# LorienLV/genarchbench

Measured on AMD Instinct MI355X. Metric: bsw ROI M alignments/sec, higher is better.
Workload: dtype i16/i32; 1 GPU; bsw-large; total_items=10000000

## Files before the change

### genarchbench_amd/csrc/bsw.hip

```cpp
#include "gab_internal.h"
#include <atomic>
#include <algorithm>
#include <new>
#include <string.h>
#include <time.h>
#include <stdlib.h>

namespace {

constexpr int kQBuckets = 256;
constexpr int kTBuckets = 256;
constexpr int kNumKeys = kQBuckets * kTBuckets;
constexpr int kClassStep = 16;
constexpr int kNumClasses = kQBuckets / kClassStep;

struct BswConst {
    int32_t o_del, e_del, o_ins, e_ins, zdrop, end_bonus, w, max_sc;
    uint32_t row_lo[5];
    uint32_t row_hi[5];
};

struct BswStats {
    unsigned long long cells;
    int32_t max_h0[kNumClasses];
    int32_t bad;
    int32_t first_bad;
};
GAB_STATIC_ATOMIC64(BswStats, cells);

struct BswIO {
    const uint8_t *ref; const int64_t *ref_off;
    const uint8_t *qry; const int64_t *qry_off;
    const int32_t *len1, *len2, *h0;
    int64_t ref_bytes, qry_bytes, n;
    int64_t ref_lo, qry_lo;
    int64_t ref_hi, qry_hi;
};

__device__ __forceinline__ int bsw_key(int qlen, int tlen, int h0) {
    int tb = tlen >> 3; if (tb > kTBuckets / 4 - 1) tb = kTBuckets / 4 - 1;
    int hc = h0 >> 5; if (hc > 3) hc = 3;
    return (qlen - 1) * kTBuckets + tb * 4 + hc;
}

__device__ __forceinline__ int bsw_hslot(int key) { return (int)(((uint32_t)key * 4099u) & (uint32_t)(kNumKeys - 1)); }
static_assert((kNumKeys & (kNumKeys - 1)) == 0, "bsw_hslot needs a power-of-two key space");

__global__ __launch_bounds__(256) void bsw_hist(BswIO io, uint32_t *hist, uint32_t *rank, BswStats *st) {
    __shared__ int cls_h0[kNumClasses];
    if (threadIdx.x < kNumClasses) cls_h0[threadIdx.x] = 0;
    __syncthreads();
    int64_t i = (int64_t)blockIdx.x * blockDim.x + threadIdx.x;
    int64_t stride = (int64_t)gridDim.x * blockDim.x;
    for (; i < io.n; i += stride) {
        int ql = io.len2[i], tl = io.len1[i], h = io.h0[i];
        int64_t ro = io.ref_off[i], qo = io.qry_off[i];
        bool ok = ql >= 1 && ql <= GAB_BSW_MAX_QLEN && tl >= 1 && tl <= GAB_BSW_MAX_TLEN && h >= 0 &&
                  h <= (1 << 29) && ro >= io.ref_lo && qo >= io.qry_lo &&
                  ro + tl + 3 <= io.ref_bytes && qo + ql + 3 <= io.qry_bytes &&
                  ro + tl <= io.ref_hi && qo + ql <= io.qry_hi;
        if (!ok) {
            atomicAdd(&st->bad, 1);
            atomicMin((unsigned int *)&st->first_bad, (unsigned int)(i + 1 > 0x7fffffff ? 0x7fffffff : i + 1));
            rank[i] = ~0u;
            continue;
        }
        if (h > 0) atomicMax(&cls_h0[(ql - 1) / kClassStep], h);
        rank[i] = atomicAdd(&hist[bsw_hslot(bsw_key(ql, tl, h))], 1u);
    }
    __syncthreads();
    if (threadIdx.x < kNumClasses && cls_h0[threadIdx.x] > 0) atomicMax(&st->max_h0[threadIdx.x], cls_h0[threadIdx.x]);
}

constexpr int kScanBlocks = kNumKeys / 1024;
static_assert(kScanBlocks == 64, "bsw_scan_b reduces the block totals with one wave");
__global__ __launch_bounds__(1024) void bsw_scan_a(const uint32_t *__restrict__ hist, uint32_t *__restrict__ start, uint32_t *__restrict__ sums) {
    __shared__ uint32_t wsum[16];
    const int t = threadIdx.x, key = blockIdx.x * 1024 + t, lane = t & 63, wv = t >> 6;
    const uint32_t v = hist[bsw_hslot(key)];
    uint32_t inc = v;
    for (int o = 1; o < 64; o <<= 1) { const uint32_t u = __shfl_up(inc, o); if (lane >= o) inc += u; }
    if (lane == 63) wsum[wv] = inc;
    __syncthreads();
    uint32_t before = 0;
    for (int k = 0; k < wv; k++) before += wsum[k];
    start[key] = before + inc - v;
    if (t == 1023) sums[blockIdx.x] = before + inc;
}
__global__ __launch_bounds__(1024) void bsw_scan_b(uint32_t *__restrict__ start, const uint32_t *__restrict__ sums, uint32_t *__restrict__ qstart) {
    __shared__ uint32_t s_off, s_total;
    const int t = threadIdx.x, key = blockIdx.x * 1024 + t;
    if (t < 64) {
        const uint32_t sv = sums[t];
        uint32_t mine = t < (int)blockIdx.x ? sv : 0, all = sv;
        for (int o = 32; o > 0; o >>= 1) { mine += __shfl_xor(mine, o); all += __shfl_xor(all, o); }
        if (t == 0) { s_off = mine; s_total = all; }
    }
    __syncthreads();
    const uint32_t run = start[key] + s_off;
    start[key] = run;
    if ((key % kTBuckets) == 0) qstart[key / kTBuckets] = run;
    if (key == kNumKeys - 1) { start[kNumKeys] = s_total; qstart[kQBuckets] = s_total; }
}

struct __attribute__((aligned(32))) BswRec { int64_t ref_off, qry_off; int32_t len1, len2, h0; uint32_t id; };

__global__ __launch_bounds__(256) void bsw_scatter(BswIO io, const uint32_t *__restrict__ start, const uint32_t *__restrict__ rank,
                                                   BswRec *recs) {
    int64_t i = (int64_t)blockIdx.x * blockDim.x + threadIdx.x;
    int64_t stride = (int64_t)gridDim.x * blockDim.x;
    for (; i < io.n; i += stride) {
        int ql = io.len2[i], tl = io.len1[i];
        if (rank[i] == ~0u) continue;
        BswRec r;
        r.ref_off = io.ref_off[i]; r.qry_off = io.qry_off[i]; r.len1 = tl; r.len2 = ql; r.h0 = io.h0[i]; r.id = (uint32_t)i;
        recs[start[bsw_key(ql, tl, r.h0)] + rank[i]] = r;
    }
}

__device__ __forceinline__ uint32_t load_u32_unaligned(const uint8_t *p) {
    uint32_t w;
    __builtin_memcpy(&w, p, 4);
    return w;
}

template <bool WIDE>
__global__ __launch_bounds__(64) void bsw_dp(BswIO io, BswConst c, const BswRec *__restrict__ recs,
                                            int64_t kbeg, int64_t kend, int qcap,
                                            int32_t *__restrict__ score_out,
                                            gab_bsw_result *__restrict__ result_out, BswStats *st) {
    extern __shared__ uint32_t lds[];
    const int lane = threadIdx.x;
    const int64_t k = kbeg + (int64_t)(gridDim.x - 1 - blockIdx.x) * 64 + lane;
    const bool valid = k < kend;
    BswRec rec; rec.ref_off = rec.qry_off = 0; rec.len1 = rec.len2 = rec.h0 = 0; rec.id = 0u;
    if (valid) rec = recs[k];
    const uint32_t id = rec.id;

    uint32_t *const H = lds + lane;
    uint32_t *const E = lds + (size_t)(qcap + 1) * 64 + lane;
    uint8_t *const QC = reinterpret_cast<uint8_t *>(lds + (size_t)(WIDE ? 2 : 1) * (qcap + 1) * 64) + lane * 4;

    unsigned long long cells = 0;
    if (valid) {
        const int qlen = rec.len2, tlen = rec.len1, h0 = rec.h0;
        const uint8_t *q = io.qry + rec.qry_off;
        const uint8_t *t = io.ref + rec.ref_off;
        const int oe_del = c.o_del + c.e_del, oe_ins = c.o_ins + c.e_ins;
        const int e_del = c.e_del, e_ins = c.e_ins;

        for (int w4 = 0; w4 * 4 < qlen; w4++)
            *reinterpret_cast<uint32_t *>(QC + w4 * 256) = load_u32_unaligned(q + w4 * 4);

        int w = c.w;
        {
            int lim = (int)((double)(qlen * c.max_sc + c.end_bonus - c.o_ins) / e_ins + 1.);
            lim = lim > 1 ? lim : 1; w = w < lim ? w : lim;
            lim = (int)((double)(qlen * c.max_sc + c.end_bonus - c.o_del) / e_del + 1.);
            lim = lim > 1 ? lim : 1; w = w < lim ? w : lim;
        }
        const bool score_only = result_out == nullptr;
        bool prune = score_only && (qlen <= w + 1 || h0 - oe_ins - (w + 1) * e_ins <= 0) && (c.zdrop == 0 || c.zdrop >= 8 * c.max_sc);
        int best, best_i, best_j, g_i, gscore, max_off;
      for (;;) {
// ... 512 lines not shown
                    uint32_t cl2 = (uint32_t)(qlen - 2 * pb) | (uint32_t)(qlen - 2 * pb - 1) << 16;
                    uint32_t acc = 0;
                    for (int p = pb; p <= pe; p++, cl2 -= 0x00020002u) {
                        uint32_t d2 = CW[p * 64] & 0x00ff00ffu;
                        if (p == pb && (beg & 1)) d2 &= 0xffff0000u;
                        if (p == pe && !(end & 1)) d2 &= 0x0000ffffu;
                        const uint32_t gain = pk_mul_lo(pk_min_u16(cl2, r2), m2);
                        acc = pk_max_i16(acc, pk_mul_lo(add_u32_v(d2, gain), pk_min_u16_1(d2)));
                    }
                    bound = max(bound, max((int)(acc & 0xffffu), (int)(acc >> 16)));
                }
                stop = bound <= best;
            }
            if (stop) break;
        }
        if (!SO || !abandon) break;
        prune = false;
      }
        score_out[id] = best;
        if constexpr (!SO) {
            gab_bsw_result r;
            r.score = best; r.qle = best_j + 1; r.tle = best_i + 1;
            r.gtle = g_i + 1; r.gscore = gscore; r.max_off = max_off;
            result_out[id] = r;
        }
    }
#undef CELL16
#undef QPAIR
    for (int o = 32; o > 0; o >>= 1) cells += __shfl_xor(cells, o);
    if (lane == 0 && cells) atomicAdd(&st->cells, cells);
}

using BswDp8Fn = void (*)(BswIO, BswConst, const BswRec *, int64_t, int64_t, int, int32_t *, gab_bsw_result *, BswStats *);
template <bool SYM, bool MS1> BswDp8Fn bsw_dp8_pick(bool so) { return so ? bsw_dp8<SYM, MS1, true> : bsw_dp8<SYM, MS1, false>; }
BswDp8Fn bsw_dp8_kernel(bool sym, bool ms1, bool so) {
    return sym ? (ms1 ? bsw_dp8_pick<true, true>(so) : bsw_dp8_pick<true, false>(so))
               : (ms1 ? bsw_dp8_pick<false, true>(so) : bsw_dp8_pick<false, false>(so));
}

}

struct gab_bsw {
    gab_tuning tun = gab_tuning_loaded();
    gab_host_stream hs;
    int device = 0;
    gab_bsw_params prm;
    BswConst cst;
    gab_devbuf ws;
    gab_devbuf io;
    hipEvent_t ev[4] = {nullptr, nullptr, nullptr, nullptr};
    static constexpr int kAux = 1;
    hipStream_t aux[kAux] = {nullptr};
    hipEvent_t fork = nullptr, join[kAux] = {nullptr};
    bool have_stats = false;
    uint32_t *h_qstart = nullptr;
    BswStats *h_stats = nullptr;
    int64_t last_cells = 0;
    bool out_of_order = false;
};

extern "C" int gab_bsw_create(const gab_bsw_params *p, int device, gab_bsw **out) {
    if (!p || !out) { gab_set_error("gab_bsw_create: NULL argument"); return GAB_EINVAL; }
    *out = nullptr;
    GAB_CHECK(p->e_del > 0 && p->e_ins > 0 && p->o_del >= 0 && p->o_ins >= 0,
              "gab_bsw_create: gap penalties must be o>=0, e>0 (got o_del=%d e_del=%d o_ins=%d e_ins=%d)",
              p->o_del, p->e_del, p->o_ins, p->e_ins);
    GAB_CHECK(p->w >= 0 && p->zdrop >= 0, "gab_bsw_create: w and zdrop must be >= 0");
    GAB_CHECK(p->o_del + p->e_del < 32768 && p->o_ins + p->e_ins < 32768 && p->end_bonus >= -32768 &&
              p->end_bonus < 32768, "gab_bsw_create: penalties out of 16-bit range");
    int rc = gab_check_device(device);
    if (rc) return rc;
    gab_device_guard g(device);
    gab_bsw *h = new (std::nothrow) gab_bsw();
    if (!h) { gab_set_error("out of host memory"); return GAB_ENOMEM; }
    h->device = device; h->prm = *p;
    BswConst &c = h->cst;
    c.o_del = p->o_del; c.e_del = p->e_del; c.o_ins = p->o_ins; c.e_ins = p->e_ins;
    c.zdrop = p->zdrop; c.end_bonus = p->end_bonus; c.w = p->w;
    int mx = 0;
    for (int k = 0; k < 25; k++) mx = p->mat[k] > mx ? p->mat[k] : mx;
    c.max_sc = mx;
    for (int t = 0; t < 5; t++) {
        uint32_t lo = 0;
        for (int q = 0; q < 4; q++) lo |= (uint32_t)(uint8_t)(p->mat[t * 5 + q] + 128) << (8 * q);
        c.row_lo[t] = lo;
        c.row_hi[t] = (uint32_t)(uint8_t)(p->mat[t * 5 + 4] + 128);
    }
    for (int k = 0; k < 4; k++)
        if (hipEventCreate(&h->ev[k]) != hipSuccess) { gab_set_error("hipEventCreate failed"); delete h; return GAB_EDEVICE; }
    bool aux_ok = hipEventCreateWithFlags(&h->fork, hipEventDisableTiming) == hipSuccess;
    for (int k = 0; k < gab_bsw::kAux && aux_ok; k++)
        aux_ok = hipStreamCreateWithFlags(&h->aux[k], hipStreamNonBlocking) == hipSuccess &&
                 hipEventCreateWithFlags(&h->join[k], hipEventDisableTiming) == hipSuccess;
    if (!aux_ok) { gab_set_error("gab_bsw_create: stream / event creation failed"); delete h; return GAB_EDEVICE; }
    if (hipFuncSetAttribute((const void *)bsw_dp<false>, hipFuncAttributeMaxDynamicSharedMemorySize, 160 * 1024) != hipSuccess ||
        hipFuncSetAttribute((const void *)bsw_dp<true>, hipFuncAttributeMaxDynamicSharedMemorySize, 160 * 1024) != hipSuccess) {
        gab_set_error("hipFuncSetAttribute(MaxDynamicSharedMemorySize) failed"); delete h; return GAB_EDEVICE;
    }
    for (int k = 0; k < 8; k++)
        if (hipFuncSetAttribute((const void *)bsw_dp8_kernel(k & 4, k & 2, k & 1), hipFuncAttributeMaxDynamicSharedMemorySize, 160 * 1024 - 64) != hipSuccess) {
            gab_set_error("hipFuncSetAttribute(MaxDynamicSharedMemorySize) failed"); delete h; return GAB_EDEVICE;
        }
    if (hipHostMalloc((void **)&h->h_qstart, sizeof(uint32_t) * (kQBuckets + 1)) != hipSuccess ||
        hipHostMalloc((void **)&h->h_stats, sizeof(BswStats)) != hipSuccess) {
        gab_set_error("hipHostMalloc failed"); delete h; return GAB_ENOMEM;
    }
    *out = h;
    return GAB_OK;
}

extern "C" void gab_bsw_destroy(gab_bsw *h) {
    if (!h) return;
    gab_device_guard g(h->device);
    h->ws.release(); h->io.release(); h->hs.release();
    for (int k = 0; k < 4; k++) if (h->ev[k]) (void)hipEventDestroy(h->ev[k]);
    if (h->fork) (void)hipEventDestroy(h->fork);
    for (int k = 0; k < gab_bsw::kAux; k++) {
        if (h->join[k]) (void)hipEventDestroy(h->join[k]);
        if (h->aux[k]) (void)hipStreamDestroy(h->aux[k]);
    }
    if (h->h_qstart) (void)hipHostFree(h->h_qstart);
    if (h->h_stats) (void)hipHostFree(h->h_stats);
    delete h;
}

static int bsw_run_device_impl(gab_bsw *h, const uint8_t *ref, int64_t ref_bytes, const int64_t *ref_off,
                               const uint8_t *qry, int64_t qry_bytes, const int64_t *qry_off,
                               const int32_t *len1, const int32_t *len2, const int32_t *h0, int64_t n,
                               int32_t *score_out, gab_bsw_result *result_out, void *stream_, int64_t ref_lo, int64_t qry_lo,
                               int64_t ref_hi, int64_t qry_hi);
extern "C" int gab_bsw_run_device(gab_bsw *h, const uint8_t *ref, int64_t ref_bytes, const int64_t *ref_off,
                                  const uint8_t *qry, int64_t qry_bytes, const int64_t *qry_off,
                                  const int32_t *len1, const int32_t *len2, const int32_t *h0, int64_t n,
                                  int32_t *score_out, gab_bsw_result *result_out, void *stream_) {
    if (h) gab_tuning_refresh(&h->tun);
    return bsw_run_device_impl(h, ref, ref_bytes, ref_off, qry, qry_bytes, qry_off, len1, len2, h0, n, score_out, result_out, stream_, 0, 0,
                               ref_bytes, qry_bytes);
}
static int bsw_run_device_impl(gab_bsw *h, const uint8_t *ref, int64_t ref_bytes, const int64_t *ref_off,
                               const uint8_t *qry, int64_t qry_bytes, const int64_t *qry_off,
                               const int32_t *len1, const int32_t *len2, const int32_t *h0, int64_t n,
                               int32_t *score_out, gab_bsw_result *result_out, void *stream_, int64_t ref_lo, int64_t qry_lo,
                               int64_t ref_hi, int64_t qry_hi) {
    GAB_CHECK(h, "gab_bsw_run_device: NULL handle");
    GAB_CHECK(n >= 0 && n < (1ll << 31), "gab_bsw_run_device: n=%lld out of range", (long long)n);
    h->have_stats = false;
    if (n == 0) return GAB_OK;
    GAB_CHECK(ref && ref_off && qry && qry_off && len1 && len2 && h0 && score_out,
              "gab_bsw_run_device: NULL buffer");
    gab_device_guard g(h->device);
    hipStream_t s = (hipStream_t)stream_;

    const size_t o_hist = 0;
    const size_t o_start = o_hist + sizeof(uint32_t) * kNumKeys;
    const size_t o_qstart = o_start + sizeof(uint32_t) * (kNumKeys + 1);
    const size_t o_sums = o_qstart + sizeof(uint32_t) * (kQBuckets + 1);
    const size_t o_stats = (o_sums + sizeof(uint32_t) * kScanBlocks + 15) & ~(size_t)15;
    const size_t o_recs = (o_stats + sizeof(BswStats) + 255) & ~(size_t)255;
    const size_t o_rank = o_recs + ((sizeof(BswRec) * (size_t)n + 255) & ~(size_t)255);
    int rc = h->ws.reserve(o_rank + sizeof(uint32_t) * (size_t)n);
    if (rc) return rc;
    char *base = h->ws.as<char>();
    uint32_t *d_hist = (uint32_t *)(base + o_hist), *d_start = (uint32_t *)(base + o_start);
    uint32_t *d_qstart = (uint32_t *)(base + o_qstart);
    BswStats *d_stats = (BswStats *)(base + o_stats);
    BswRec *d_recs = (BswRec *)(base + o_recs);
    uint32_t *d_rank = (uint32_t *)(base + o_rank);

    BswIO io{ref, ref_off, qry, qry_off, len1, len2, h0, ref_bytes, qry_bytes, n, ref_lo, qry_lo, ref_hi, qry_hi};
    GAB_HIP(hipEventRecord(h->ev[0], s));
    GAB_HIP(hipMemsetAsync(base, 0, o_recs, s));
    {
        BswStats init; memset(&init, 0, sizeof(init)); init.first_bad = 0x7fffffff;
        *h->h_stats = init;
        GAB_HIP(hipMemcpyAsync(d_stats, h->h_stats, sizeof(BswStats), hipMemcpyHostToDevice, s));
    }
    int grid = (int)(gab_ceil_div(n, 256) < 1024 ? gab_ceil_div(n, 256) : 1024);
    hipLaunchKernelGGL(bsw_hist, dim3(grid), dim3(256), 0, s, io, d_hist, d_rank, d_stats);
    hipLaunchKernelGGL(bsw_scan_a, dim3(kScanBlocks), dim3(1024), 0, s, d_hist, d_start, (uint32_t *)(base + o_sums));
    hipLaunchKernelGGL(bsw_scan_b, dim3(kScanBlocks), dim3(1024), 0, s, d_start, (const uint32_t *)(base + o_sums), d_qstart);
    hipLaunchKernelGGL(bsw_scatter, dim3(grid), dim3(256), 0, s, io, d_start, d_rank, d_recs);
    GAB_HIP(hipMemcpyAsync(h->h_qstart, d_qstart, sizeof(uint32_t) * (kQBuckets + 1), hipMemcpyDeviceToHost, s));
    GAB_HIP(hipMemcpyAsync(h->h_stats, d_stats, sizeof(BswStats), hipMemcpyDeviceToHost, s));
    GAB_HIP(hipStreamSynchronize(s));
    if (h->h_stats->bad) {
        gab_set_error("gab_bsw_run_device: %d pair(s) violate the limits (first: pair %d): need 1<=len2<=%d, "
                      "1<=len1<=%d, 0<=h0, offsets inside the slabs with 3 more readable bytes behind every sequence",
                      h->h_stats->bad, h->h_stats->first_bad - 1, GAB_BSW_MAX_QLEN, GAB_BSW_MAX_TLEN);
        return GAB_EINVAL;
    }
    int max_h0 = 0;
    for (int cls = 0; cls < kNumClasses; cls++) max_h0 = h->h_stats->max_h0[cls] > max_h0 ? h->h_stats->max_h0[cls] : max_h0;
    const bool sym = h->cst.o_del + h->cst.e_del == h->cst.o_ins + h->cst.e_ins;
    const bool ms1 = h->cst.max_sc <= 1;

    GAB_HIP(hipEventRecord(h->ev[1], s));
    GAB_HIP(hipEventRecord(h->fork, s));
    for (int k = 0; k < gab_bsw::kAux; k++) GAB_HIP(hipStreamWaitEvent(h->aux[k], h->fork, 0));
    int nlaunch = 0;
    hipStream_t s_main = s;
    const bool one_launch = n <= (int64_t)64 * 8192;
    int top_cls = kNumClasses - 1;
    while (top_cls > 0 && h->h_qstart[(top_cls + 1) * kClassStep] <= h->h_qstart[top_cls * kClassStep]) top_cls--;
    for (int cls = kNumClasses - 1; cls >= 0; cls--) {
        int64_t kb = h->h_qstart[cls * kClassStep], ke = h->h_qstart[(cls + 1) * kClassStep];
        if (one_launch) { if (cls != top_cls) continue; kb = 0; }
        if (ke <= kb) continue;
        const int qcap = (cls + 1) * kClassStep;
        const int blocks = (int)gab_ceil_div(ke - kb, 64);
        s = (nlaunch % (gab_bsw::kAux + 1)) ? h->aux[nlaunch % (gab_bsw::kAux + 1) - 1] : s_main;
        nlaunch++;
        const int64_t hmax = (int64_t)(one_launch ? max_h0 : h->h_stats->max_h0[cls]) + (int64_t)qcap * h->cst.max_sc;
        const bool wide = hmax > 32767;
        if (h->tun.bsw_trace)
            fprintf(stderr, "[gab_bsw_dp %p] class %d qcap %d pairs %lld bits %d sym %d ms1 %d\n", (void *)h, cls, qcap,
                    (long long)(ke - kb), hmax <= 255 ? 8 : wide ? 32 : 16, (int)sym, (int)ms1);
        if (hmax <= 255 && h->cst.max_sc >= 0) {
            const size_t lds8 = sizeof(uint32_t) * 64 * ((size_t)(qcap + 2) / 2 + ((size_t)(qcap + 1) / 2 + 3) / 4 + 1);
            auto kern = bsw_dp8_kernel(sym, ms1, result_out == nullptr);
            hipLaunchKernelGGL(kern, dim3(blocks), dim3(64), lds8, s, io, h->cst, d_recs, kb, ke, qcap,
                               score_out, result_out, d_stats);
            continue;
        }
        const size_t lds = sizeof(uint32_t) * 64 * ((size_t)(wide ? 2 : 1) * (qcap + 1) + (size_t)(qcap + 3) / 4);
        if (wide)
            hipLaunchKernelGGL(bsw_dp<true>, dim3(blocks), dim3(64), lds, s, io, h->cst, d_recs, kb, ke, qcap,
                               score_out, result_out, d_stats);
        else
            hipLaunchKernelGGL(bsw_dp<false>, dim3(blocks), dim3(64), lds, s, io, h->cst, d_recs, kb, ke, qcap,
                               score_out, result_out, d_stats);
    }
    s = s_main;
    GAB_HIP(hipGetLastError());
    for (int k = 0; k < gab_bsw::kAux; k++) {
        GAB_HIP(hipEventRecord(h->join[k], h->aux[k]));
        GAB_HIP(hipStreamWaitEvent(s, h->join[k], 0));
    }
    GAB_HIP(hipEventRecord(h->ev[2], s));
    GAB_HIP(hipMemcpyAsync(h->h_stats, d_stats, sizeof(BswStats), hipMemcpyDeviceToHost, s));
    GAB_HIP(hipEventRecord(h->ev[3], s));
    h->have_stats = true;
    return GAB_OK;
}

extern "C" int gab_bsw_run(gab_bsw *h, const uint8_t *ref, const int64_t *ref_off, const uint8_t *qry,
                           const int64_t *qry_off, const int32_t *len1, const int32_t *len2,
                           const int32_t *h0, int64_t n, int32_t *score_out) {
    GAB_CHECK(h, "gab_bsw_run: NULL handle");
    GAB_CHECK(n >= 0 && n < (1ll << 31), "gab_bsw_run: n=%lld out of range", (long long)n);
    if (n == 0) return GAB_OK;
    GAB_CHECK(ref && ref_off && qry && qry_off && len1 && len2 && h0 && score_out, "gab_bsw_run: NULL buffer");
    gab_device_guard g(h->device);
    gab_tuning_refresh(&h->tun);
    const bool trace = h->tun.bsw_trace;
    const double t_0 = gab_now_ms();
    int64_t rb = 0, qb = 0, ra = INT64_MAX, qa = INT64_MAX;
    auto take = [&](int64_t i) {
        int64_t r = ref_off[i] + len1[i], q = qry_off[i] + len2[i];
        rb = r > rb ? r : rb; qb = q > qb ? q : qb;
        ra = ref_off[i] < ra ? ref_off[i] : ra; qa = qry_off[i] < qa ? qry_off[i] : qa;
        return ref_off[i] >= 0 && qry_off[i] >= 0 && len1[i] >= 0 && len2[i] >= 0;
    };
    bool sampled = n > 4096 && !h->out_of_order && !h->tun.bsw_full_scan;
    if (sampled) {
        bool ok = take(0);
        ok = take(n - 1) && ok;
        for (int k = 1; k <= 64; k++) ok = take((n - 1) * k / 65) && ok;
        if (!ok || rb - ra > 65536 * n || qb - qa > 65536 * n) sampled = false;
    }
    if (!sampled) {
        rb = qb = 0; ra = qa = INT64_MAX;
        for (int64_t i = 0; i < n; i++)
            GAB_CHECK(take(i), "gab_bsw_run: negative offset/length at pair %lld", (long long)i);
    }
    ra &= ~(int64_t)255; qa &= ~(int64_t)255;
    const size_t rpad = ((size_t)(rb - ra) + 3 + 255) & ~(size_t)255, qpad = ((size_t)(qb - qa) + 3 + 255) & ~(size_t)255;
    const size_t nn = (size_t)n;
    size_t o = 0;
    const size_t o_ref = o; o += rpad;
    const size_t o_qry = o; o += qpad;
    const size_t o_roff = o; o += 8 * nn;
    const size_t o_qoff = o; o += 8 * nn;
    const size_t o_l1 = o; o += 4 * nn;
    const size_t o_l2 = o; o += 4 * nn;
    const size_t o_h0 = o; o += 4 * nn;
    const size_t o_sc = o; o += 4 * nn;
    int rc = h->io.reserve(o);
    if (rc) return rc;
    char *b = h->io.as<char>();
    hipStream_t s = nullptr;
    if ((rc = h->hs.get(&s)) != GAB_OK) return rc;
    const double t_1 = gab_now_ms();
    {
        std::lock_guard<std::mutex> gate(gab_h2d_mutex(h->device));
        GAB_HIP(hipMemcpyAsync(b + o_ref, ref + ra, (size_t)(rb - ra), hipMemcpyHostToDevice, s));
        GAB_HIP(hipMemcpyAsync(b + o_qry, qry + qa, (size_t)(qb - qa), hipMemcpyHostToDevice, s));
        GAB_HIP(hipMemcpyAsync(b + o_roff, ref_off, 8 * nn, hipMemcpyHostToDevice, s));
        GAB_HIP(hipMemcpyAsync(b + o_qoff, qry_off, 8 * nn, hipMemcpyHostToDevice, s));
        GAB_HIP(hipMemcpyAsync(b + o_l1, len1, 4 * nn, hipMemcpyHostToDevice, s));
        GAB_HIP(hipMemcpyAsync(b + o_l2, len2, 4 * nn, hipMemcpyHostToDevice, s));
        GAB_HIP(hipMemcpyAsync(b + o_h0, h0, 4 * nn, hipMemcpyHostToDevice, s));
        GAB_HIP(hipStreamSynchronize(s));
    }
    double t_2 = 0;
    if (trace) { GAB_HIP(hipStreamSynchronize(s)); t_2 = gab_now_ms(); }
    rc = bsw_run_device_impl(h, (const uint8_t *)(b + o_ref) - ra, ra + (int64_t)rpad, (const int64_t *)(b + o_roff),
                             (const uint8_t *)(b + o_qry) - qa, qa + (int64_t)qpad, (const int64_t *)(b + o_qoff),
                             (const int32_t *)(b + o_l1), (const int32_t *)(b + o_l2), (const int32_t *)(b + o_h0),
                             n, (int32_t *)(b + o_sc), nullptr, s, ra, qa, rb, qb);
    if (rc == GAB_EINVAL && sampled) {
        h->out_of_order = true;
        return gab_bsw_run(h, ref, ref_off, qry, qry_off, len1, len2, h0, n, score_out);
    }
    if (rc) return rc;
    double t_3 = 0;
    if (trace) { GAB_HIP(hipStreamSynchronize(s)); t_3 = gab_now_ms(); }
    GAB_HIP(hipMemcpyAsync(score_out, b + o_sc, 4 * nn, hipMemcpyDeviceToHost, s));
    GAB_HIP(hipStreamSynchronize(s));
    if (trace)
        fprintf(stderr, "[gab_bsw_run %p] %lld pairs: host scan %.2f ms, H2D of %.1f MB %.2f ms, sort + DP %.2f ms, D2H %.2f ms\n", (void *)h,
                (long long)n, t_1 - t_0, (double)((rb - ra) + (qb - qa) + 28 * n) / 1e6, t_2 - t_1, t_3 - t_2, gab_now_ms() - t_3);
    return GAB_OK;
}

extern "C" int gab_bsw_reserve(gab_bsw *h, int64_t max_pairs, int64_t max_ref_bytes, int64_t max_qry_bytes) {
    GAB_CHECK(h, "gab_bsw_reserve: NULL handle");
    GAB_CHECK(max_pairs >= 0 && max_pairs < (1ll << 31) && max_ref_bytes >= 0 && max_qry_bytes >= 0, "gab_bsw_reserve: size out of range");
    gab_device_guard g(h->device);
    const size_t nn = (size_t)max_pairs;
    int rc = h->io.reserve(std::max<size_t>((((size_t)max_ref_bytes + 3 + 511) & ~(size_t)255) + (((size_t)max_qry_bytes + 3 + 511) & ~(size_t)255) + 32 * nn + 1024,
                                            (size_t)4 << 20));
    if (rc) return rc;
    rc = h->ws.reserve(sizeof(uint32_t) * (2 * kNumKeys + kQBuckets + 4) + sizeof(BswStats) + 1024 + (sizeof(BswRec) + sizeof(uint32_t)) * nn);
    if (rc) return rc;
    hipStream_t s = nullptr;
    if ((rc = h->hs.get(&s)) != GAB_OK) return rc;
    GAB_HIP(hipMemsetAsync(h->io.p, 0, h->io.cap, s));
    GAB_HIP(hipMemsetAsync(h->ws.p, 0, h->ws.cap, s));
    GAB_HIP(hipStreamSynchronize(s));
    if ((rc = gab_warm_copy_engines(s, h->io.p, h->io.cap)) != GAB_OK) return rc;
    static const uint8_t seq[40] = {0, 1, 2, 3, 0, 1, 2, 3, 3, 2, 1, 0, 0, 1, 2, 3, 0, 1, 2, 3, 3, 2, 1, 0, 0, 1, 2, 3, 0, 1, 2, 3, 3, 2, 1, 0, 0, 0, 0, 0};
    const int64_t ro[2] = {0, 4}, qo[2] = {2, 8};
    const int32_t l1[2] = {24, 20}, l2[2] = {20, 16}, h0[2] = {10, 0};
    int32_t sc[2];
    const bool had = h->have_stats;
    rc = gab_bsw_run(h, seq, ro, seq, qo, l1, l2, h0, 2, sc);
    h->have_stats = had;
    return rc;
}

extern "C" int gab_bsw_last_stats(gab_bsw *h, int64_t *cells, float *kernel_ms, float *total_ms) {
    GAB_CHECK(h, "gab_bsw_last_stats: NULL handle");
    GAB_CHECK(h->have_stats, "gab_bsw_last_stats: no completed run on this handle");
    gab_device_guard g(h->device);
    GAB_HIP(hipEventSynchronize(h->ev[3]));
    if (cells) *cells = (int64_t)h->h_stats->cells;
    if (kernel_ms) GAB_HIP(hipEventElapsedTime(kernel_ms, h->ev[1], h->ev[2]));
    if (total_ms) GAB_HIP(hipEventElapsedTime(total_ms, h->ev[0], h->ev[3]));
    return GAB_OK;
}
```

### genarchbench_amd/csrc/gab_core.hip

```cpp
#define GAB_NO_COPY_MACROS
#include "gab_internal.h"
#include <string.h>
#include <stdlib.h>
#include <algorithm>
#include <mutex>
#include <unordered_set>

static thread_local char g_err[512] = "";

void gab_set_error(const char *fmt, ...) {
    va_list ap;
    va_start(ap, fmt);
    vsnprintf(g_err, sizeof(g_err), fmt, ap);
    va_end(ap);
}

extern "C" const char *gab_version(void) { return "gab-hip 0.1 (gfx950)"; }

#include <execinfo.h>
#include <fcntl.h>
#include <signal.h>
#include <sys/stat.h>
#include <unistd.h>
namespace {
// ... 29 lines not shown
}
extern "C" const char *gab_last_error(void) { return g_err; }

extern "C" int gab_device_count(void) {
    int n = 0;
    if (hipGetDeviceCount(&n) != hipSuccess) return 0;
    return n;
}

extern "C" int gab_device_pci_bus_id(int device, char *buf, int len) {
    if (!buf || len < 16) { gab_set_error("gab_device_pci_bus_id: buffer of at least 16 bytes needed"); return GAB_EINVAL; }
    buf[0] = 0;
    const int n = gab_device_count();
    if (n <= 0) { gab_set_error("no HIP device visible"); return GAB_ENODEV; }
    if (device < 0 || device >= n) { gab_set_error("device %d out of range (0..%d)", device, n - 1); return GAB_EINVAL; }
    GAB_HIP(hipDeviceGetPCIBusId(buf, len, device));
    return GAB_OK;
}

int gab_check_device(int device) {
    int n = gab_device_count();
    if (n <= 0) {
        gab_set_error("no HIP device visible (libgab_hip has no CPU fallback)");
        return GAB_ENODEV;
    }
    if (device < 0 || device >= n) {
        gab_set_error("device %d out of range (0..%d)", device, n - 1);
        return GAB_EINVAL;
    }
    hipDeviceProp_t prop;
    if (hipGetDeviceProperties(&prop, device) != hipSuccess) {
        gab_set_error("hipGetDeviceProperties(%d) failed", device);
        return GAB_EDEVICE;
    }
    if (const char *e = getenv("GAB_HIP_SCHEDULE")) {
        static std::once_flag once;
        std::call_once(once, [e] {
            (void)hipSetDeviceFlags(!strcmp(e, "spin") ? hipDeviceScheduleSpin : !strcmp(e, "yield") ? hipDeviceScheduleYield : hipDeviceScheduleBlockingSync);
        });
    }
    if (strncmp(prop.gcnArchName, "gfx950", 6) != 0) {
        gab_set_error("device %d is %s; this library is built for gfx950 only", device, prop.gcnArchName);
        return GAB_ENODEV;
    }
    return GAB_OK;
}

bool gab_tuning_live() { const char *e = getenv("GAB_TUNING_LIVE"); return e && *e && atoi(e) != 0; }
void gab_tuning_load(gab_tuning *t) {
    *t = gab_tuning();
    auto on = [](const char *name) { return getenv(name) != nullptr; };
    auto num = [](const char *name, long long unset) { const char *e = getenv(name); return e ? atoll(e) : unset; };
    t->bsw_trace = on("GAB_BSW_TRACE"); t->bsw_full_scan = on("GAB_BSW_FULL_SCAN");
    t->bpm_score64 = on("GAB_BPM_SCORE64"); t->bitpal_no_bv = on("GAB_BITPAL_NO_BV"); t->bpm_slices = (int)num("GAB_BPM_SLICES", 0);
    t->bpm_trace = on("GAB_BPM_TRACE");
    if (const char *e = getenv("GAB_WFA_TUNE")) {
        t->wfa_tuned = true;
        const int k = sscanf(e, "%d,%d,%d,%d,%d,%d,%d", &t->wfa_tune[0], &t->wfa_tune[1], &t->wfa_tune[2], &t->wfa_tune[3], &t->wfa_tune[4], &t->wfa_tune[5], &t->wfa_tune[6]);
        t->wfa_tune_fields = k > 0 ? k : 0;
    }
    t->wfa_no_static = on("GAB_WFA_NO_STATIC"); t->wfa_trace = on("GAB_WFA_TRACE");
    t->wfa_pool2 = (int)num("GAB_WFA_POOL2", -1); t->wfa_slots = (int)num("GAB_WFA_SLOTS", -1);
    if (const char *e = getenv("GAB_CHAIN_HELPERS")) { t->chain_helpers_set = true; t->chain_helpers = atoi(e); }
    { const char *e = getenv("GAB_CHAIN_KERNEL"); t->chain_walk = e && !strcmp(e, "walk"); }
    t->chain_trace = on("GAB_CHAIN_TRACE"); t->chain_feed_giveup = on("GAB_CHAIN_FEED_GIVEUP"); t->chain_fed_serial = on("GAB_CHAIN_FED_SERIAL");
    t->chain_no_overlap = on("GAB_CHAIN_NO_OVERLAP"); t->chain_no_feed = on("GAB_CHAIN_NO_FEED");
    if (const char *e = getenv("GAB_CHAIN_TAB")) t->chain_tab = atoi(e) != 0;
    t->chain_tab_min = num("GAB_CHAIN_TAB_MIN", -1); t->chain_fast_min = num("GAB_CHAIN_FAST_MIN", -1); t->chain_fast_calls = num("GAB_CHAIN_FAST_CALLS", -1);
    t->chain_feed_min = num("GAB_CHAIN_FEED_MIN", -1); t->chain_tab_mb = num("GAB_CHAIN_TAB_MB", -1);
    if (const char *e = getenv("GAB_CHAIN_GATHER_MASK")) { strncpy(t->chain_gather_mask, e, sizeof t->chain_gather_mask - 1); t->chain_gather_mask[sizeof t->chain_gather_mask - 1] = 0; }
    t->chain_gather_blocks = (int)num("GAB_CHAIN_GATHER_BLOCKS", 0);
    t->fmi_lds_entries = (int)num("GAB_FMI_LDS_ENTRIES", 0); t->fmi_waves = (int)num("GAB_FMI_WAVES", 0); t->fmi_wide = (int)num("GAB_FMI_WIDE", 1);
    t->fmi_wide_cap = (int)num("GAB_FMI_WIDE_CAP", 0); t->fmi_kmer_depth = (int)num("GAB_FMI_KMER_DEPTH", -1);
    t->fmi_wide_lists = num("GAB_FMI_WIDE_LISTS", 0) != 0; t->fmi_debug = on("GAB_FMI_DEBUG");
    t->fmi_batch = num("GAB_FMI_BATCH", 0); t->fmi_scratch_mb = num("GAB_FMI_SCRATCH_MB", 0);
    t->kmer_part_floor = num("GAB_KMER_PART_FLOOR", 0) != 0;
    t->abea_trace_bytes = num("GAB_ABEA_TRACE_BYTES", 0);
}

extern "C" int gab_device_alloc(int device, size_t bytes, void **out) {
    if (!out) { gab_set_error("gab_device_alloc: NULL argument"); return GAB_EINVAL; }
    *out = nullptr;
    int rc = gab_check_device(device);
    if (rc) return rc;
    gab_device_guard g(device);
    GAB_HIP(hipMalloc(out, bytes ? bytes : 1));
    return GAB_OK;
}
extern "C" void gab_device_free(int device, void *p) {
    if (!p) return;
    gab_device_guard g(device);
    (void)hipFree(p);
}
extern "C" int gab_device_copy_to_host(int device, void *dst, const void *d_src, size_t bytes) {
    if (bytes == 0) return GAB_OK;
    if (!dst || !d_src) { gab_set_error("gab_device_copy_to_host: NULL argument"); return GAB_EINVAL; }
    gab_device_guard g(device);
    GAB_HIP(gab_memcpy_async(dst, d_src, bytes, hipMemcpyDeviceToHost, nullptr));
    GAB_HIP(hipStreamSynchronize(nullptr));
    return GAB_OK;
}

static std::mutex g_host_mu;
static std::unordered_set<void *> &gab_host_blocks() { static std::unordered_set<void *> s; return s; }
extern "C" int gab_host_alloc(size_t bytes, void **out) {
    if (!out) { gab_set_error("gab_host_alloc: NULL argument"); return GAB_EINVAL; }
// ... 123 lines not shown
```

### genarchbench_amd/csrc/gab_internal.h

```cpp
#pragma once
#include <hip/hip_runtime.h>
#include <stdint.h>
#include <stdarg.h>
#include <stdio.h>
#include <stddef.h>
#include <time.h>
#include <mutex>
#include "../../include/gab.h"

void gab_set_error(const char *fmt, ...);

#define GAB_HIP(call)                                                                    \
    do {                                                                                 \
        hipError_t e_ = (call);                                                          \
        if (e_ != hipSuccess) {                                                          \
            gab_set_error("%s:%d: %s -> %s", __FILE__, __LINE__, #call,                  \
                          hipGetErrorString(e_));                                        \
            return e_ == hipErrorOutOfMemory ? GAB_ENOMEM : GAB_EDEVICE;                 \
        }                                                                                \
    } while (0)

#define GAB_CHECK(cond, ...)                                                             \
    do {                                                                                 \
        if (!(cond)) {                                                                   \
// ... 4 lines not shown

struct gab_devbuf {
    void *p = nullptr;
    size_t cap = 0;
    int reserve(size_t bytes) {
        if (bytes <= cap) return GAB_OK;
        if (p) (void)hipFree(p);
        p = nullptr; cap = 0;
        size_t want = bytes + bytes / 8 + 256;
        hipError_t e = hipMalloc(&p, want);
        if (e != hipSuccess) {
            gab_set_error("hipMalloc(%zu) failed: %s", want, hipGetErrorString(e));
            p = nullptr;
            return GAB_ENOMEM;
        }
        cap = want;
        return GAB_OK;
    }
    void release() { if (p) (void)hipFree(p); p = nullptr; cap = 0; }
    template <typename T> T *as() const { return reinterpret_cast<T *>(p); }
};

struct gab_device_guard {
    int prev = -1; bool changed = false;
    explicit gab_device_guard(int dev) {
        if (hipGetDevice(&prev) == hipSuccess && prev != dev) { changed = (hipSetDevice(dev) == hipSuccess); }
    }
    ~gab_device_guard() { if (changed) (void)hipSetDevice(prev); }
};

struct gab_host_stream {
    hipStream_t s = nullptr;
    int get(hipStream_t *out) {
        if (!s && hipStreamCreateWithFlags(&s, hipStreamNonBlocking) != hipSuccess) {
            s = nullptr; gab_set_error("hipStreamCreateWithFlags failed: %s", hipGetErrorString(hipGetLastError()));
            return GAB_EDEVICE;
        }
        *out = s;
        return GAB_OK;
    }
    void release() { if (s) (void)hipStreamDestroy(s); s = nullptr; }
};

std::mutex &gab_h2d_mutex(int device);
int gab_warm_copy_engines(hipStream_t s, void *dev, size_t dev_bytes);
int gab_check_device(int device);
bool gab_is_pinned(const void *p);

static inline int64_t gab_ceil_div(int64_t a, int64_t b) { return (a + b - 1) / b; }
static inline double gab_now_ms() { timespec ts; clock_gettime(CLOCK_MONOTONIC, &ts); return ts.tv_sec * 1e3 + ts.tv_nsec * 1e-6; }

struct gab_tuning {
    bool bsw_trace = false, bsw_full_scan = false;
    bool bpm_score64 = false, bitpal_no_bv = false, bpm_trace = false;
    int bpm_slices = 0;
    bool wfa_tuned = false, wfa_no_static = false, wfa_trace = false;
    int wfa_tune[7] = {0, 0, 0, 0, 0, 0, 0};
    int wfa_tune_fields = 0;
    int wfa_pool2 = -1, wfa_slots = -1;
    int chain_helpers = 0;
    bool chain_helpers_set = false, chain_walk = false, chain_trace = false, chain_feed_giveup = false, chain_fed_serial = false;
    bool chain_no_overlap = false, chain_no_feed = false;
    int chain_tab = -1;
    long long chain_tab_min = -1, chain_fast_min = -1, chain_fast_calls = -1, chain_feed_min = -1, chain_tab_mb = -1;
    char chain_gather_mask[32] = "";
    int chain_gather_blocks = 0;
    int fmi_lds_entries = 0, fmi_waves = 0, fmi_wide = 1, fmi_wide_cap = 0, fmi_kmer_depth = -1;
    bool fmi_wide_lists = false, fmi_debug = false;
    long long fmi_batch = 0, fmi_scratch_mb = 0;
    bool kmer_part_floor = false;
    long long abea_trace_bytes = 0;
};
void gab_tuning_load(gab_tuning *t);
bool gab_tuning_live();
inline void gab_tuning_refresh(gab_tuning *t) { if (gab_tuning_live()) gab_tuning_load(t); }
inline gab_tuning gab_tuning_loaded() { gab_tuning t; gab_tuning_load(&t); return t; }

#define GAB_CHECK_ATOMIC64(off) GAB_CHECK((((size_t)(off)) & 7) == 0, "internal error: a 64-bit atomic at offset %zu of a scratch layout (not a multiple of 8)", (size_t)(off))
#define GAB_STATIC_ATOMIC64(type, member) static_assert(offsetof(type, member) % 8 == 0 && alignof(type) >= 8, "64-bit atomics need 8-byte alignment: " #type "::" #member)

__device__ __forceinline__ uint32_t gab_wave_slot(uint32_t *counter, bool active) {
    const unsigned long long m = __ballot(active);
    if (!m) return 0;
    const int lane = (int)(threadIdx.x & 63u);
    const int leader = __builtin_ctzll(m);
    uint32_t base = 0;
    if (lane == leader) base = atomicAdd(counter, (uint32_t)__popcll(m));
    base = __shfl(base, leader);
    return base + (uint32_t)__popcll(m & ((1ull << lane) - 1ull));
}

hipError_t gab_memcpy_async(void *dst, const void *src, size_t bytes, hipMemcpyKind kind, hipStream_t s);
hipError_t gab_memcpy(void *dst, const void *src, size_t bytes, hipMemcpyKind kind);
#ifndef GAB_NO_COPY_MACROS
#define hipMemcpyAsync gab_memcpy_async
#define hipMemcpy gab_memcpy
#endif
```

Baseline: 400.1 M alignments/s.

## Slice BSW input and overlap second slice's sort with first slice's DP

```diff
diff --git a/genarchbench_amd/csrc/bsw.hip b/genarchbench_amd/csrc/bsw.hip
--- a/genarchbench_amd/csrc/bsw.hip
+++ b/genarchbench_amd/csrc/bsw.hip
@@ -13,6 +13,11 @@
 constexpr int kNumKeys = kQBuckets * kTBuckets;
 constexpr int kClassStep = 16;
 constexpr int kNumClasses = kQBuckets / kClassStep;
+constexpr int kSlices = 2;
+constexpr int64_t kSlice0 = 1 << 20;
+constexpr int64_t kSliceMin = 1 << 22;
+constexpr int kSortGridBeside = 256;
+static_assert(kSliceMin >= (1 << 21) && kSlice0 < kSliceMin && kSlice0 >= 64 * 8192, "slice 0 has to fill the chip with its class launches, and calls below 2^21 pairs stay unsliced");
 
 struct BswConst {
     int32_t o_del, e_del, o_ins, e_ins, zdrop, end_bonus, w, max_sc;
@@ -46,13 +51,13 @@
 __device__ __forceinline__ int bsw_hslot(int key) { return (int)(((uint32_t)key * 4099u) & (uint32_t)(kNumKeys - 1)); }
 static_assert((kNumKeys & (kNumKeys - 1)) == 0, "bsw_hslot needs a power-of-two key space");
 
-__global__ __launch_bounds__(256) void bsw_hist(BswIO io, uint32_t *hist, uint32_t *rank, BswStats *st) {
+__global__ __launch_bounds__(256) void bsw_hist(BswIO io, int64_t lo, int64_t hi, uint32_t *hist, uint32_t *rank, BswStats *st) {
     __shared__ int cls_h0[kNumClasses];
     if (threadIdx.x < kNumClasses) cls_h0[threadIdx.x] = 0;
     __syncthreads();
-    int64_t i = (int64_t)blockIdx.x * blockDim.x + threadIdx.x;
+    int64_t i = lo + (int64_t)blockIdx.x * blockDim.x + threadIdx.x;
     int64_t stride = (int64_t)gridDim.x * blockDim.x;
-    for (; i < io.n; i += stride) {
+    for (; i < hi; i += stride) {
         int ql = io.len2[i], tl = io.len1[i], h = io.h0[i];
         int64_t ro = io.ref_off[i], qo = io.qry_off[i];
         bool ok = ql >= 1 && ql <= GAB_BSW_MAX_QLEN && tl >= 1 && tl <= GAB_BSW_MAX_TLEN && h >= 0 &&
@@ -105,11 +110,11 @@
 
 struct __attribute__((aligned(32))) BswRec { int64_t ref_off, qry_off; int32_t len1, len2, h0; uint32_t id; };
 
-__global__ __launch_bounds__(256) void bsw_scatter(BswIO io, const uint32_t *__restrict__ start, const uint32_t *__restrict__ rank,
-                                                   BswRec *recs) {
-    int64_t i = (int64_t)blockIdx.x * blockDim.x + threadIdx.x;
+__global__ __launch_bounds__(256) void bsw_scatter(BswIO io, int64_t lo, int64_t hi, const uint32_t *__restrict__ start,
+                                                   const uint32_t *__restrict__ rank, BswRec *recs) {
+    int64_t i = lo + (int64_t)blockIdx.x * blockDim.x + threadIdx.x;
     int64_t stride = (int64_t)gridDim.x * blockDim.x;
-    for (; i < io.n; i += stride) {
+    for (; i < hi; i += stride) {
         int ql = io.len2[i], tl = io.len1[i];
         if (rank[i] == ~0u) continue;
         BswRec r;
@@ -728,10 +733,13 @@
     static constexpr int kAux = 1;
     hipStream_t aux[kAux] = {nullptr};
     hipEvent_t fork = nullptr, join[kAux] = {nullptr};
+    hipStream_t sort = nullptr;
+    hipEvent_t sort_fork = nullptr, sort_join = nullptr;
     bool have_stats = false;
-    uint32_t *h_qstart = nullptr;
-    BswStats *h_stats = nullptr;
-    int64_t last_cells = 0;
+    int stat_slices = 1;
+    uint32_t *h_qstart[kSlices] = {nullptr};
+    BswStats *h_stats[kSlices] = {nullptr};
+    BswStats *h_init = nullptr;
     bool out_of_order = false;
 };
 
@@ -777,10 +785,14 @@
         if (hipFuncSetAttribute((const void *)bsw_dp8_kernel(k & 4, k & 2, k & 1), hipFuncAttributeMaxDynamicSharedMemorySize, 160 * 1024 - 64) != hipSuccess) {
             gab_set_error("hipFuncSetAttribute(MaxDynamicSharedMemorySize) failed"); delete h; return GAB_EDEVICE;
         }
-    if (hipHostMalloc((void **)&h->h_qstart, sizeof(uint32_t) * (kQBuckets + 1)) != hipSuccess ||
-        hipHostMalloc((void **)&h->h_stats, sizeof(BswStats)) != hipSuccess) {
-        gab_set_error("hipHostMalloc failed"); delete h; return GAB_ENOMEM;
-    }
+    if (hipHostMalloc((void **)&h->h_qstart[0], sizeof(uint32_t) * (kQBuckets + 1) * kSlices) != hipSuccess ||
+        hipHostMalloc((void **)&h->h_stats[0], sizeof(BswStats) * (kSlices + 1)) != hipSuccess) {
+        gab_set_error("hipHostMalloc failed"); gab_bsw_destroy(h); return GAB_ENOMEM;
+    }
+    for (int k = 1; k < kSlices; k++) { h->h_qstart[k] = h->h_qstart[0] + (size_t)k * (kQBuckets + 1); h->h_stats[k] = h->h_stats[0] + k; }
+    h->h_init = h->h_stats[0] + kSlices;
+    memset(h->h_init, 0, sizeof(BswStats));
+    h->h_init->first_bad = 0x7fffffff;
     *out = h;
     return GAB_OK;
 }
@@ -795,10 +807,28 @@
         if (h->join[k]) (void)hipEventDestroy(h->join[k]);
         if (h->aux[k]) (void)hipStreamDestroy(h->aux[k]);
     }
-    if (h->h_qstart) (void)hipHostFree(h->h_qstart);
-    if (h->h_stats) (void)hipHostFree(h->h_stats);
+    if (h->sort_fork) (void)hipEventDestroy(h->sort_fork);
+    if (h->sort_join) (void)hipEventDestroy(h->sort_join);
+    if (h->sort) (void)hipStreamDestroy(h->sort);
+    if (h->h_qstart[0]) (void)hipHostFree(h->h_qstart[0]);
+    if (h->h_stats[0]) (void)hipHostFree(h->h_stats[0]);
     delete h;
 }
+
+struct BswLayout {
+    size_t o_start, o_qstart, o_sums, o_stats, blk;
+    size_t o_recs, o_rank, total;
+    explicit BswLayout(size_t n) {
+        o_start = sizeof(uint32_t) * kNumKeys;
+        o_qstart = o_start + sizeof(uint32_t) * (kNumKeys + 1);
+        o_sums = o_qstart + sizeof(uint32_t) * (kQBuckets + 1);
+        o_stats = (o_sums + sizeof(uint32_t) * kScanBlocks + 15) & ~(size_t)15;
+        blk = (o_stats + sizeof(BswStats) + 255) & ~(size_t)255;
+        o_recs = blk * kSlices;
+        o_rank = o_recs + ((sizeof(BswRec) * n + 255) & ~(size_t)255);
+        total = o_rank + sizeof(uint32_t) * n;
+    }
+};
 
 static int bsw_run_device_impl(gab_bsw *h, const uint8_t *ref, int64_t ref_bytes, const int64_t *ref_off,
                                const uint8_t *qry, int64_t qry_bytes, const int64_t *qry_off,
@@ -827,94 +857,153 @@
     gab_device_guard g(h->device);
     hipStream_t s = (hipStream_t)stream_;
 
-    const size_t o_hist = 0;
-    const size_t o_start = o_hist + sizeof(uint32_t) * kNumKeys;
-    const size_t o_qstart = o_start + sizeof(uint32_t) * (kNumKeys + 1);
-    const size_t o_sums = o_qstart + sizeof(uint32_t) * (kQBuckets + 1);
-    const size_t o_stats = (o_sums + sizeof(uint32_t) * kScanBlocks + 15) & ~(size_t)15;
-    const size_t o_recs = (o_stats + sizeof(BswStats) + 255) & ~(size_t)255;
-    const size_t o_rank = o_recs + ((sizeof(BswRec) * (size_t)n + 255) & ~(size_t)255);
-    int rc = h->ws.reserve(o_rank + sizeof(uint32_t) * (size_t)n);
+    const int64_t slice0 = h->tun.bsw_slice[0] > 0 ? h->tun.bsw_slice[0] : kSlice0;
+    const int64_t slice_min = std::max<int64_t>(h->tun.bsw_slice[1] > 0 ? h->tun.bsw_slice[1] : kSliceMin, slice0 + 1);
+    const int nsl = n >= slice_min ? kSlices : 1;
+    const int64_t cut[kSlices + 1] = {0, nsl > 1 ? slice0 : n, n};
+    if (nsl > 1 && !h->sort) {
+        if (hipStreamCreateWithFlags(&h->sort, hipStreamNonBlocking) != hipSuccess) { h->sort = nullptr; gab_set_error("gab_bsw_run_device: stream creation failed"); return GAB_EDEVICE; }
+        if (!h->sort_fork) GAB_HIP(hipEventCreateWithFlags(&h->sort_fork, hipEventDisableTiming));
+        if (!h->sort_join) GAB_HIP(hipEventCreateWithFlags(&h->sort_join, hipEventDisableTiming));
+    }
+
+    const BswLayout L((size_t)n);
+    int rc = h->ws.reserve(L.total);
     if (rc) return rc;
     char *base = h->ws.as<char>();
-    uint32_t *d_hist = (uint32_t *)(base + o_hist), *d_start = (uint32_t *)(base + o_start);
-    uint32_t *d_qstart = (uint32_t *)(base + o_qstart);
-    BswStats *d_stats = (BswStats *)(base + o_stats);
-    BswRec *d_recs = (BswRec *)(base + o_recs);
-    uint32_t *d_rank = (uint32_t *)(base + o_rank);
+    BswRec *d_recs = (BswRec *)(base + L.o_recs);
+    uint32_t *d_rank = (uint32_t *)(base + L.o_rank);
+    auto d_stats = [&](int k) { return (BswStats *)(base + L.blk * k + L.o_stats); };
 
     BswIO io{ref, ref_off, qry, qry_off, len1, len2, h0, ref_bytes, qry_bytes, n, ref_lo, qry_lo, ref_hi, qry_hi};
+    auto enqueue_sort = [&](int k, hipStream_t q) -> hipError_t {
+        char *b = base + L.blk * k;
+        uint32_t *d_hist = (uint32_t *)b, *d_start = (uint32_t *)(b + L.o_start), *d_qstart = (uint32_t *)(b + L.o_qstart);
+        uint32_t *d_sums = (uint32_t *)(b + L.o_sums);
+        const int64_t lo = cut[k], hi = cut[k + 1];
+        hipError_t e = hipMemsetAsync(b, 0, L.blk, q);
+        if (e == hipSuccess) e = hipMemcpyAsync(d_stats(k), h->h_init, sizeof(BswStats), hipMemcpyHostToDevice, q);
+        if (e != hipSuccess) return e;
+        const int gmax = k > 0 ? kSortGridBeside : 1024;
+        const int grid = (int)(gab_ceil_div(hi - lo, 256) < gmax ? gab_ceil_div(hi - lo, 256) : gmax);
+        hipLaunchKernelGGL(bsw_hist, dim3(grid), dim3(256), 0, q, io, lo, hi, d_hist, d_rank, d_stats(k));
+        hipLaunchKernelGGL(bsw_scan_a, dim3(kScanBlocks), dim3(1024), 0, q, d_hist, d_start, d_sums);
+        hipLaunchKernelGGL(bsw_scan_b, dim3(kScanBlocks), dim3(1024), 0, q, d_start, (const uint32_t *)d_sums, d_qstart);
+        hipLaunchKernelGGL(bsw_scatter, dim3(grid), dim3(256), 0, q, io, lo, hi, d_start, d_rank, d_recs + lo);
+        e = hipMemcpyAsync(h->h_qstart[k], d_qstart, sizeof(uint32_t) * (kQBuckets + 1), hipMemcpyDeviceToHost, q);
+        if (e == hipSuccess) e = hipMemcpyAsync(h->h_stats[k], d_stats(k), sizeof(BswStats), hipMemcpyDeviceToHost, q);
+        return e;
+    };
     GAB_HIP(hipEventRecord(h->ev[0], s));
-    GAB_HIP(hipMemsetAsync(base, 0, o_recs, s));
-    {
-        BswStats init; memset(&init, 0, sizeof(init)); init.first_bad = 0x7fffffff;
-        *h->h_stats = init;
-        GAB_HIP(hipMemcpyAsync(d_stats, h->h_stats, sizeof(BswStats), hipMemcpyHostToDevice, s));
-    }
-    int grid = (int)(gab_ceil_div(n, 256) < 1024 ? gab_ceil_div(n, 256) : 1024);
-    hipLaunchKernelGGL(bsw_hist, dim3(grid), dim3(256), 0, s, io, d_hist, d_rank, d_stats);
-    hipLaunchKernelGGL(bsw_scan_a, dim3(kScanBlocks), dim3(1024), 0, s, d_hist, d_start, (uint32_t *)(base + o_sums));
-    hipLaunchKernelGGL(bsw_scan_b, dim3(kScanBlocks), dim3(1024), 0, s, d_start, (const uint32_t *)(base + o_sums), d_qstart);
-    hipLaunchKernelGGL(bsw_scatter, dim3(grid), dim3(256), 0, s, io, d_start, d_rank, d_recs);
-    GAB_HIP(hipMemcpyAsync(h->h_qstart, d_qstart, sizeof(uint32_t) * (kQBuckets + 1), hipMemcpyDeviceToHost, s));
-    GAB_HIP(hipMemcpyAsync(h->h_stats, d_stats, sizeof(BswStats), hipMemcpyDeviceToHost, s));
+    GAB_HIP(enqueue_sort(0, s));
     GAB_HIP(hipStreamSynchronize(s));
-    if (h->h_stats->bad) {
-        gab_set_error("gab_bsw_run_device: %d pair(s) violate the limits (first: pair %d): need 1<=len2<=%d, "
-                      "1<=len1<=%d, 0<=h0, offsets inside the slabs with 3 more readable bytes behind every sequence",
-                      h->h_stats->bad, h->h_stats->first_bad - 1, GAB_BSW_MAX_QLEN, GAB_BSW_MAX_TLEN);
-        return GAB_EINVAL;
-    }
-    int max_h0 = 0;
-    for (int cls = 0; cls < kNumClasses; cls++) max_h0 = h->h_stats->max_h0[cls] > max_h0 ? h->h_stats->max_h0[cls] : max_h0;
     const bool sym = h->cst.o_del + h->cst.e_del == h->cst.o_ins + h->cst.e_ins;
     const bool ms1 = h->cst.max_sc <= 1;
 
-    GAB_HIP(hipEventRecord(h->ev[1], s));
+    hipStream_t s_main = s;
+    auto join_all = [&]() {
+        (void)hipStreamSynchronize(s_main);
+        for (int k = 0; k < gab_bsw::kAux; k++) (void)hipStreamSynchronize(h->aux[k]);
+        if (nsl > 1) (void)hipStreamSynchronize(h->sort);
+    };
+#define BSW_HIP_JOINED(call)                                                                                       \
+    do {                                                                                                           \
+        hipError_t e_ = (call);                                                                                    \
+        if (e_ != hipSuccess) {                                                                                    \
+            gab_set_error("%s:%d: %s -> %s", __FILE__, __LINE__, #call, hipGetErrorString(e_));                    \
+            join_all();                                                                                            \
+            return e_ == hipErrorOutOfMemory ? GAB_ENOMEM : GAB_EDEVICE;                                           \
+        }                                                                                                          \
+    } while (0)
     GAB_HIP(hipEventRecord(h->fork, s));
     for (int k = 0; k < gab_bsw::kAux; k++) GAB_HIP(hipStreamWaitEvent(h->aux[k], h->fork, 0));
     int nlaunch = 0;
-    hipStream_t s_main = s;
-    const bool one_launch = n <= (int64_t)64 * 8192;
+    constexpr int kRing = gab_bsw::kAux + 2;
+    hipStream_t ring[kRing] = {nsl > 1 ? h->sort : nullptr, s_main};
+    for (int k = 0; k < gab_bsw::kAux; k++) ring[k + 2] = h->aux[k];
+    for (int sl = 0; sl < nsl; sl++) {
+    if (sl > 0) BSW_HIP_JOINED(hipStreamSynchronize(h->sort));
+    const BswStats &hst = *h->h_stats[sl];
+    const uint32_t *qstart = h->h_qstart[sl];
+    if (hst.bad) {
+        gab_set_error("gab_bsw_run_device: %d pair(s) violate the limits (first: pair %d): need 1<=len2<=%d, "
+                      "1<=len1<=%d, 0<=h0, offsets inside the slabs with 3 more readable bytes behind every sequence",
+                      hst.bad, hst.first_bad - 1, GAB_BSW_MAX_QLEN, GAB_BSW_MAX_TLEN);
+        join_all();
+        return GAB_EINVAL;
+    }
+    const bool last = sl + 1 == nsl;
+    if (!last) {
+        BSW_HIP_JOINED(hipEventRecord(h->sort_fork, s_main));
+        BSW_HIP_JOINED(hipStreamWaitEvent(h->sort, h->sort_fork, 0));
+        BSW_HIP_JOINED(enqueue_sort(sl + 1, h->sort));
+    }
+    if (sl == 0) BSW_HIP_JOINED(hipEventRecord(h->ev[1], s));
+    int max_h0 = 0;
+    for (int cls = 0; cls < kNumClasses; cls++) max_h0 = hst.max_h0[cls] > max_h0 ? hst.max_h0[cls] : max_h0;
+    char slice_tag[16] = "";
+    if (nsl > 1) snprintf(slice_tag, sizeof slice_tag, " slice %d", sl);
+    const bool one_launch = nsl == 1 && n <= (int64_t)64 * 8192;
     int top_cls = kNumClasses - 1;
-    while (top_cls > 0 && h->h_qstart[(top_cls + 1) * kClassStep] <= h->h_qstart[top_cls * kClassStep]) top_cls--;
+    while (top_cls > 0 && qstart[(top_cls + 1) * kClassStep] <= qstart[top_cls * kClassStep]) top_cls--;
+    int ring_phase = 0;
+    if (sl > 0) {
+        int64_t heaviest = 0;
+        for (int cls = kNumClasses - 1, k = 0; cls >= 0 && k < kRing; cls--) {
+            const int64_t w = ((int64_t)qstart[(cls + 1) * kClassStep] - (int64_t)qstart[cls * kClassStep]) * (cls + 1);
+            if (w <= 0) continue;
+            if (w > heaviest) { heaviest = w; ring_phase = k; }
+            k++;
+        }
+        nlaunch = 0;
+    }
     for (int cls = kNumClasses - 1; cls >= 0; cls--) {
-        int64_t kb = h->h_qstart[cls * kClassStep], ke = h->h_qstart[(cls + 1) * kClassStep];
+        int64_t kb = qstart[cls * kClassStep], ke = qstart[(cls + 1) * kClassStep];
         if (one_launch) { if (cls != top_cls) continue; kb = 0; }
         if (ke <= kb) continue;
         const int qcap = (cls + 1) * kClassStep;
         const int blocks = (int)gab_ceil_div(ke - kb, 64);
         s = (nlaunch % (gab_bsw::kAux + 1)) ? h->aux[nlaunch % (gab_bsw::kAux + 1) - 1] : s_main;
+        if (sl > 0) s = ring[(nlaunch - ring_phase + kRing) % kRing];
         nlaunch++;
-        const int64_t hmax = (int64_t)(one_launch ? max_h0 : h->h_stats->max_h0[cls]) + (int64_t)qcap * h->cst.max_sc;
+        const int64_t hmax = (int64_t)(one_launch ? max_h0 : hst.max_h0[cls]) + (int64_t)qcap * h->cst.max_sc;
         const bool wide = hmax > 32767;
         if (h->tun.bsw_trace)
-            fprintf(stderr, "[gab_bsw_dp %p] class %d qcap %d pairs %lld bits %d sym %d ms1 %d\n", (void *)h, cls, qcap,
-                    (long long)(ke - kb), hmax <= 255 ? 8 : wide ? 32 : 16, (int)sym, (int)ms1);
+            fprintf(stderr, "[gab_bsw_dp %p] class %d qcap %d pairs %lld bits %d sym %d ms1 %d%s\n", (void *)h, cls, qcap,
+                    (long long)(ke - kb), hmax <= 255 ? 8 : wide ? 32 : 16, (int)sym, (int)ms1, slice_tag);
+        kb += cut[sl]; ke += cut[sl];
+        BswStats *const d_st = d_stats(sl);
         if (hmax <= 255 && h->cst.max_sc >= 0) {
             const size_t lds8 = sizeof(uint32_t) * 64 * ((size_t)(qcap + 2) / 2 + ((size_t)(qcap + 1) / 2 + 3) / 4 + 1);
             auto kern = bsw_dp8_kernel(sym, ms1, result_out == nullptr);
             hipLaunchKernelGGL(kern, dim3(blocks), dim3(64), lds8, s, io, h->cst, d_recs, kb, ke, qcap,
-                               score_out, result_out, d_stats);
+                               score_out, result_out, d_st);
             continue;
         }
         const size_t lds = sizeof(uint32_t) * 64 * ((size_t)(wide ? 2 : 1) * (qcap + 1) + (size_t)(qcap + 3) / 4);
         if (wide)
             hipLaunchKernelGGL(bsw_dp<true>, dim3(blocks), dim3(64), lds, s, io, h->cst, d_recs, kb, ke, qcap,
-                               score_out, result_out, d_stats);
+                               score_out, result_out, d_st);
         else
             hipLaunchKernelGGL(bsw_dp<false>, dim3(blocks), dim3(64), lds, s, io, h->cst, d_recs, kb, ke, qcap,
-                               score_out, result_out, d_stats);
+                               score_out, result_out, d_st);
     }
     s = s_main;
-    GAB_HIP(hipGetLastError());
+    BSW_HIP_JOINED(hipGetLastError());
+    }
+    if (nsl > 1) {
+        BSW_HIP_JOINED(hipEventRecord(h->sort_join, h->sort));
+        BSW_HIP_JOINED(hipStreamWaitEvent(s, h->sort_join, 0));
+    }
     for (int k = 0; k < gab_bsw::kAux; k++) {
-        GAB_HIP(hipEventRecord(h->join[k], h->aux[k]));
-        GAB_HIP(hipStreamWaitEvent(s, h->join[k], 0));
-    }
-    GAB_HIP(hipEventRecord(h->ev[2], s));
-    GAB_HIP(hipMemcpyAsync(h->h_stats, d_stats, sizeof(BswStats), hipMemcpyDeviceToHost, s));
-    GAB_HIP(hipEventRecord(h->ev[3], s));
+        BSW_HIP_JOINED(hipEventRecord(h->join[k], h->aux[k]));
+        BSW_HIP_JOINED(hipStreamWaitEvent(s, h->join[k], 0));
+    }
+    BSW_HIP_JOINED(hipEventRecord(h->ev[2], s));
+    for (int k = 0; k < nsl; k++) BSW_HIP_JOINED(hipMemcpyAsync(h->h_stats[k], d_stats(k), sizeof(BswStats), hipMemcpyDeviceToHost, s));
+    BSW_HIP_JOINED(hipEventRecord(h->ev[3], s));
+#undef BSW_HIP_JOINED
+    h->stat_slices = nsl;
     h->have_stats = true;
     return GAB_OK;
 }
@@ -1007,7 +1096,7 @@
     int rc = h->io.reserve(std::max<size_t>((((size_t)max_ref_bytes + 3 + 511) & ~(size_t)255) + (((size_t)max_qry_bytes + 3 + 511) & ~(size_t)255) + 32 * nn + 1024,
                                             (size_t)4 << 20));
     if (rc) return rc;
-    rc = h->ws.reserve(sizeof(uint32_t) * (2 * kNumKeys + kQBuckets + 4) + sizeof(BswStats) + 1024 + (sizeof(BswRec) + sizeof(uint32_t)) * nn);
+    rc = h->ws.reserve(BswLayout(nn).total);
     if (rc) return rc;
     hipStream_t s = nullptr;
     if ((rc = h->hs.get(&s)) != GAB_OK) return rc;
@@ -1030,7 +1119,10 @@
     GAB_CHECK(h->have_stats, "gab_bsw_last_stats: no completed run on this handle");
     gab_device_guard g(h->device);
     GAB_HIP(hipEventSynchronize(h->ev[3]));
-    if (cells) *cells = (int64_t)h->h_stats->cells;
+    if (cells) {
+        *cells = 0;
+        for (int k = 0; k < h->stat_slices; k++) *cells += (int64_t)h->h_stats[k]->cells;
+    }
     if (kernel_ms) GAB_HIP(hipEventElapsedTime(kernel_ms, h->ev[1], h->ev[2]));
     if (total_ms) GAB_HIP(hipEventElapsedTime(total_ms, h->ev[0], h->ev[3]));
     return GAB_OK;
diff --git a/genarchbench_amd/csrc/gab_core.hip b/genarchbench_amd/csrc/gab_core.hip
--- a/genarchbench_amd/csrc/gab_core.hip
+++ b/genarchbench_amd/csrc/gab_core.hip
@@ -105,6 +105,11 @@
     auto on = [](const char *name) { return getenv(name) != nullptr; };
     auto num = [](const char *name, long long unset) { const char *e = getenv(name); return e ? atoll(e) : unset; };
     t->bsw_trace = on("GAB_BSW_TRACE"); t->bsw_full_scan = on("GAB_BSW_FULL_SCAN");
+    if (const char *e = getenv("GAB_BSW_SLICE")) {
+        const int k = sscanf(e, "%lld,%lld", &t->bsw_slice[0], &t->bsw_slice[1]);
+        if (k < 2) t->bsw_slice[1] = -1;
+        if (k < 1) t->bsw_slice[0] = -1;
+    }
     t->bpm_score64 = on("GAB_BPM_SCORE64"); t->bitpal_no_bv = on("GAB_BITPAL_NO_BV"); t->bpm_slices = (int)num("GAB_BPM_SLICES", 0);
     t->bpm_trace = on("GAB_BPM_TRACE");
     if (const char *e = getenv("GAB_WFA_TUNE")) {
diff --git a/genarchbench_amd/csrc/gab_internal.h b/genarchbench_amd/csrc/gab_internal.h
--- a/genarchbench_amd/csrc/gab_internal.h
+++ b/genarchbench_amd/csrc/gab_internal.h
@@ -80,6 +80,7 @@
 
 struct gab_tuning {
     bool bsw_trace = false, bsw_full_scan = false;
+    long long bsw_slice[2] = {-1, -1};
     bool bpm_score64 = false, bitpal_no_bv = false, bpm_trace = false;
     int bpm_slices = 0;
     bool wfa_tuned = false, wfa_no_static = false, wfa_trace = false;
```

New measurement: 411.5 M alignments/s (median of 6 runs). 1.03x the previous value.
